# SensorsINI/v2e

Hardware: NVIDIA H100
Metric: Mevents/s (higher is better)
Workload: dtype fp16 tensor-core convs (fp32 accumulate) + f64 pixel state

## Files before the change

include/v2e_b200.h:

```cpp
#ifndef V2E_B200_H
#define V2E_B200_H

#include <stdint.h>

#ifdef __cplusplus
extern "C" {
#endif

typedef enum V2eStatus {
    V2E_OK = 0,
    V2E_E_INVALID = -1,
    V2E_E_CUDA = -2,
    V2E_E_CAPACITY = -3,
    V2E_E_ITER_CAP = -4,
    V2E_E_STATE = -5,
    V2E_E_UNSUPPORTED = -6,
    V2E_E_FALLBACK = -7
} V2eStatus;

typedef enum V2eFrameDtype { V2E_U8 = 0, V2E_F32 = 1, V2E_F64 = 2 } V2eFrameDtype;

const char *v2e_last_error(void);
int v2e_version(void);
int v2e_abi_info(int *version, int *emu_cfg_size, int *frame_info_size, int *unet_weights_size);
// ... 149 lines not shown
};
int v2e_conv2d_lrelu_sm100_tile(const void *x1_dev, int C1, const void *x2_dev, int C2,
                                const void *wgt_dev, const float *bias_dev, int Cout_pad, int KH, int KW,
                                int N, int H, int W, void *out_dev, int out_cstride, int out_mode,
                                int co_real, float slope, int tile, void *stream);
int v2e_conv_pick_tile(int C1, int C2, int Cout_pad, int KH, int KW, int N, int H, int W, int n_sms);

int v2e_conv2d_lrelu_sm100_strip(const void *x1_dev, int C1, const void *x2_dev, int C2,
                                 const void *wgt_row_dev, const float *bias_dev, int Cout_pad, int KH,
                                 int KW, int N, int H, int W, void *out_dev, int out_cstride,
                                 int out_mode, int co_real, float slope, void *stream);
int v2e_conv_strip_pick_kc(int C1, int C2, int Cout_pad, int KH, int KW, int W);

enum {
    V2E_STRIP_CHAIN_AUTO = -1,
    V2E_STRIP_CHAIN_PAIRED = 0,
    V2E_STRIP_CHAIN_STACKED = 1
};
int v2e_conv2d_lrelu_sm100_strip_chain(const void *x1_dev, int C1, const void *x2_dev, int C2,
                                       const void *wgt_row_dev, const float *bias_dev, int Cout_pad, int KH,
                                       int KW, int N, int H, int W, void *out_dev, int out_cstride,
                                       int out_mode, int co_real, float slope, int chain, void *stream);
int v2e_conv_strip_pick_chain(int C1, int C2, int Cout_pad, int KH, int KW, int W);

int v2e_conv2d_up2_lrelu_sm100(const void *x_low_dev, int C, const void *wgt_fold_dev, const void *wgt_plain_dev,
                               const float *bias_dev, int Cout_pad, int N, int H_out, int W_out, void *out_dev,
                               int out_cstride, float slope, void *stream);
int v2e_conv_up2_fold_weights(const float *w_host, int cout, int cin, int Cout_pad, int C_pad, void *out_host);
int v2e_conv_up2_supported_c(int C, int Cout_pad, int W_out);

typedef struct V2eUNetWeights {
    const float *w[23];
    const float *b[23];
} V2eUNetWeights;

typedef struct V2eSlomo V2eSlomo;

int v2e_slomo_create(int H, int W, int max_batch, const V2eUNetWeights *flow,
                     const V2eUNetWeights *interp, V2eSlomo **out);
int v2e_slomo_destroy(V2eSlomo *h);
int v2e_slomo_set_pairs(V2eSlomo *h, const uint8_t *frames_u8_dev, int B, void *stream);
int v2e_slomo_max_flow(V2eSlomo *h, float *max_speed_host, void *stream);
int v2e_slomo_interp(V2eSlomo *h, double t, uint8_t *out_u8_dev, float *out_f32_dev, void *stream);
int v2e_slomo_check_finite(V2eSlomo *h, int *nonfinite_host, void *stream);
int v2e_slomo_set_option(V2eSlomo *h, int option, int value);
int v2e_slomo_profile(V2eSlomo *h, int enable);
// ... 71 lines not shown
```

v2e_b200/_lib.py:

```python
import ctypes
import os

from . import build as _build

_LIB = None


class V2eEmuCfg(ctypes.Structure):
    _fields_ = [
        ("width", ctypes.c_int32), ("height", ctypes.c_int32),
        ("per_pixel_thres", ctypes.c_int32), ("hdr", ctypes.c_int32),
        ("pos_thres_nominal", ctypes.c_double), ("neg_thres_nominal", ctypes.c_double),
        ("cutoff_hz", ctypes.c_double), ("leak_rate_hz", ctypes.c_double),
        ("leak_jitter_fraction", ctypes.c_double), ("refractory_period_s", ctypes.c_double),
        ("shot_noise_rate_hz", ctypes.c_double), ("shot_inten_factor", ctypes.c_double),
        ("rng_mode", ctypes.c_int32), ("iter_cap", ctypes.c_int32),
        ("seed", ctypes.c_uint64),
        ("csdvs", ctypes.c_int32), ("max_frames_per_step", ctypes.c_int32),
        ("cs_tau_p_s", ctypes.c_double), ("cs_tau_h_s", ctypes.c_double),
        ("scidvs", ctypes.c_int32), ("photoreceptor_noise", ctypes.c_int32),
        ("rng_pixel_offset", ctypes.c_uint32), ("full_frame_px", ctypes.c_uint32),
        ("own_row0", ctypes.c_int32), ("own_rows", ctypes.c_int32),
        ("cs_halo_rows", ctypes.c_int32), ("reserved1", ctypes.c_int32),
    ]
# ... 60 lines not shown
    "v2e_emu_cs_begin": (_i, [_vp, _vp, _i, _d, _d, _u64, _u64, ctypes.POINTER(_i), _vp]),
    "v2e_emu_cs_pack": (_i, [_vp, _vp]),
    "v2e_emu_cs_unpack_from": (_i, [_vp, _vp, _vp, _vp]),
    "v2e_emu_cs_send_dev": (_vp, [_vp]),
    "v2e_emu_cs_chunk": (_i, [_vp, _i, _i, _vp]),
    "v2e_emu_cs_max_dev": (_vp, [_vp]),
    "v2e_emu_cs_advance": (_i, [_vp, _i, _i, _vp]),
    "v2e_emu_cs_update": (_i, [_vp, _vp, _i, _vp, _vp, _vp]),
    "v2e_emu_phase_filter": (_i, [_vp, _d, _d, _u64, _i, _vp]),
    "v2e_emu_read_counts": (_i, [_vp, ctypes.POINTER(ctypes.c_int32), _vp, _i, _vp]),
    "v2e_emu_phase_shot": (_i, [_vp, _vp, _i, _d, _d, _vp, _u64, _vp]),
    "v2e_emu_phase_emit": (_i, [_vp, _d, _d, _vp, _u64, _vp]),
    "v2e_conv2d_lrelu_sm100": (_i, [_vp, _i, _vp, _i, _vp, _vp, _i, _i, _i, _i, _i, _i, _vp, _i, _i, _i,
                                    ctypes.c_float, _vp]),
    "v2e_conv2d_lrelu_sm100_tile": (_i, [_vp, _i, _vp, _i, _vp, _vp, _i, _i, _i, _i, _i, _i, _vp, _i, _i, _i,
                                         ctypes.c_float, _i, _vp]),
    "v2e_conv_pick_tile": (_i, [_i, _i, _i, _i, _i, _i, _i, _i, _i]),
    "v2e_conv2d_lrelu_sm100_strip": (_i, [_vp, _i, _vp, _i, _vp, _vp, _i, _i, _i, _i, _i, _i, _vp, _i, _i, _i,
                                          ctypes.c_float, _vp]),
    "v2e_conv_strip_pick_kc": (_i, [_i, _i, _i, _i, _i, _i]),
    "v2e_conv2d_lrelu_sm100_strip_chain": (_i, [_vp, _i, _vp, _i, _vp, _vp, _i, _i, _i, _i, _i, _i, _vp, _i, _i, _i,
                                                ctypes.c_float, _i, _vp]),
    "v2e_conv_strip_pick_chain": (_i, [_i, _i, _i, _i, _i, _i]),
    "v2e_conv2d_up2_lrelu_sm100": (_i, [_vp, _i, _vp, _vp, _vp, _i, _i, _i, _i, _vp, _i, ctypes.c_float, _vp]),
    "v2e_conv_up2_fold_weights": (_i, [_vp, _i, _i, _i, _i, _vp]),
    "v2e_conv_up2_supported_c": (_i, [_i, _i, _i]),
    "v2e_slomo_create": (_i, [_i, _i, _i, _vp, _vp, ctypes.POINTER(_vp)]),
    "v2e_slomo_destroy": (_i, [_vp]),
    "v2e_slomo_set_pairs": (_i, [_vp, _vp, _i, _vp]),
    "v2e_slomo_max_flow": (_i, [_vp, ctypes.POINTER(ctypes.c_float), _vp]),
    "v2e_slomo_interp": (_i, [_vp, _d, _vp, _vp, _vp]),
    "v2e_slomo_set_option": (_i, [_vp, _i, _i]),
    "v2e_slomo_check_finite": (_i, [_vp, ctypes.POINTER(_i), _vp]),
    "v2e_slomo_profile": (_i, [_vp, _i]),
    "v2e_slomo_profile_read": (_i, [_vp, ctypes.POINTER(ctypes.c_float), ctypes.POINTER(_i),
                                    ctypes.POINTER(ctypes.c_double), _vp]),
    "v2e_slomo_profile_read_layers": (_i, [_vp, ctypes.POINTER(ctypes.c_float), ctypes.POINTER(_i),
                                           ctypes.POINTER(ctypes.c_double), ctypes.POINTER(ctypes.c_float),
                                           ctypes.POINTER(_i), ctypes.POINTER(ctypes.c_double), _vp]),
    "v2e_slomo_flow_ptr": (_vp, [_vp]),
    "v2e_slomo_intrp_ptr": (_vp, [_vp]),
    "v2e_slomo_buffer_ptr": (_vp, [_vp, _i, _i]),
    "v2e_slomo_layer_kernel": (_i, [_vp, _i, _i]),
    "v2e_resize_create": (_i, [_i, _i, _i, _i, _i, _i, ctypes.POINTER(_vp)]),
    "v2e_resize_destroy": (_i, [_vp]),
    "v2e_resize_run": (_i, [_vp, _vp, _vp, _i, _vp]),
# ... 91 lines not shown
```

v2e_b200/csrc/conv_tc.cu:

```cuda
#include <cuda.h>
#include <cuda_fp16.h>
#include <cuda_runtime.h>
#include <math.h>
#include <stdint.h>
#include <stdio.h>
#include <string.h>
#include <vector>

#include "../../include/v2e_b200.h"
#include "common.cuh"
#include "tc_common.cuh"

namespace {

constexpr int kTileH = 8, kTileW = 16, kBM = kTileH * kTileW;
constexpr int kStages = 4;
constexpr int kConvThreads = 288;
constexpr int kProducerWarp = 8;
constexpr int kConsumerWarps = 8;

struct ConvParams {
    int N, H, W;
    int C1, C2;
    int KH, KW;
// ... 213 lines not shown
#pragma unroll
            for (int i = 0; i < 2; i++) {
                const int m = 64 * (g * MH + h) + 16 * (warp & 3) + (lane >> 2) + 8 * i;
                const int py = y0 + m / kTileW, px = x0 + m % kTileW;
                inb[i] = py < p.H && px < p.W;
                pix[i] = (((size_t)n * p.H + py) * p.W + px) * p.out_cstride;
            }
#pragma unroll
            for (int j = 0; j < BN / 8; j++) {
                const int c = 8 * j + 2 * (lane & 3);
                const float2 b = __ldg((const float2 *)(bias + c));
#pragma unroll
                for (int i = 0; i < 2; i++)
                    if (inb[i])
                        *(__half2 *)(out + pix[i] + c) = __floats2half2_rn(lrelu(acc[h][4 * j + 2 * i] + b.x, p.slope),
                                                                           lrelu(acc[h][4 * j + 2 * i + 1] + b.y, p.slope));
            }
        }
    }
}


constexpr int kRowTile = 128;

struct StripParams {
    int N, H, W;
    int C1, C2;
    int KH, KW;
    int KC, BN;
    int tiles_x, seg_h, n_seg, n_items;
    int nslot;
    void *pool_out;
    int pool_cstride;
    int n_split, cout_pad;
    int slab_bytes;
    int w_bytes;
    int out_cstride, out_mode, co_real;
    float slope;
    const float *bias;
    void *out;
};
constexpr int kMaxSlot = 12;
constexpr int kStripThreads = 288;

struct RowRing {
    uint64_t *full, *empty;
    uint32_t nslot, cnt;
    int waited, released;
    __device__ __forceinline__ uint32_t slot(int i) const { return (cnt + (uint32_t)i) % nslot; }
    __device__ __forceinline__ void wait_upto(int n) {
        for (; waited < n; waited++) {
            const uint32_t g = cnt + (uint32_t)waited;
            mbar_wait(&full[g % nslot], (g / nslot) & 1u);
        }
    }
    __device__ __forceinline__ void release_upto(int n, int lane) {
        wait_upto(n);
        __syncwarp();
        for (; released < n; released++)
            if (lane == 0) mbar_arrive(&empty[slot(released)]);
    }
};

template <int KW, int KC, int BN>
__device__ __forceinline__ void strip_pair_mma(float (&acc)[2][BN / 2], const RowRing &rr, int row0, int last, int slabs,
                                                uint64_t dr, uint64_t dw, uint32_t a_off, uint32_t row16, uint32_t slab16,
// ... 30 lines not shown
                                                 uint64_t dr, uint64_t dw, uint32_t a_off, uint32_t row16, uint32_t slab16,
                                                 int rp0, int rp1) {
    constexpr int KH = KW;
    constexpr uint32_t rowb16 = (KC * 2u) >> 4, tile16 = (BN * KC * 2u) >> 4, wslab16 = stack_tiles<KW>() * tile16;
#pragma unroll
    for (int rp = rp0; rp < rp1; rp++) {
        const uint32_t a_row = rr.slot(row0 + (rp < KH ? rp : last)) * row16 + a_off;
        int sl = 0;
#pragma unroll 1
        do {
            const uint32_t a_lo = a_row + (uint32_t)sl * slab16;
            const uint32_t w_lo = (uint32_t)sl * wslab16 + (uint32_t)stack_index<KW>(rp, 0) * tile16;
#pragma unroll
            for (int s = 0; s < KW; s++) {
#pragma unroll
                for (int j = 0; j < KC / 16; j++)
                    wgmma_f16<2 * BN>(acc, desc_add(dr, a_lo + (uint32_t)s * rowb16 + 2u * j),
                                      desc_add(dw, w_lo + (uint32_t)(s * (KH + 1)) * tile16 + 2u * j), 1u);
            }
        } while (++sl < slabs);
    }
}

template <int KW, int KC, int BN, bool POOL, bool STACK>
__global__ void __launch_bounds__(kStripThreads, 1)
conv_strip_kernel(const __grid_constant__ CUtensorMap tmA, const __grid_constant__ CUtensorMap tmA2,
                  const __grid_constant__ CUtensorMap tmB, const StripParams p) {
    extern __shared__ __align__(1024) uint8_t smem_raw[];
    uint8_t *smem = align1024(smem_raw);
    __shared__ __align__(8) uint64_t full_bar[kMaxSlot], empty_bar[kMaxSlot], w_bar;

    constexpr int KH = KW, ph = KH / 2, pw = KW / 2, taps = KH * KW;
    constexpr int PW = kRowTile + KW - 1;
    constexpr uint32_t tile_bytes = BN * KC * 2;
    const int warp = threadIdx.x >> 5, lane = threadIdx.x & 31;
    const int slabs = (p.C1 + p.C2) / KC;
    const uint32_t row_bytes = (uint32_t)p.slab_bytes * slabs;
    uint8_t *ring = smem + ((p.w_bytes + 1023) & ~1023);
    const int split = (int)blockIdx.x % p.n_split, co_off = split * BN;
    const int item0 = (int)blockIdx.x / p.n_split, item_step = (int)gridDim.x / p.n_split;

    if constexpr (STACK) {
        constexpr int z_vec = (int)tile_bytes / 16, z_per_slab = KW + 1;
        for (int i = threadIdx.x; i < slabs * z_per_slab * z_vec; i += blockDim.x) {
            const int z = i / z_vec, sl = z / z_per_slab, s = z % z_per_slab;
            ((uint4 *)(smem + ((size_t)sl * stack_tiles<KW>() + (size_t)s * (KH + 1)) * tile_bytes))[i % z_vec] =
                make_uint4(0u, 0u, 0u, 0u);
        }
        fence_proxy_async();
    }
    if (threadIdx.x == 0) {
        for (int s = 0; s < p.nslot; s++) { mbar_init(&full_bar[s], 1); mbar_init(&empty_bar[s], kConsumerWarps); }
        mbar_init(&w_bar, 1);
        fence_barrier_init();
    }
    if (warp == kProducerWarp && lane == 0) {
        prefetch_tmap(&tmA);
        if (p.C2) prefetch_tmap(&tmA2);
        prefetch_tmap(&tmB);
    }
    __syncthreads();

    if (warp == kProducerWarp) {
        if (lane == 0) {
            mbar_expect_tx(&w_bar, (uint32_t)(slabs * taps) * tile_bytes);
            for (int t = 0; t < slabs * taps; t++) {
                const int sl = t / taps, tap = t % taps;
                const int dst = STACK ? sl * stack_tiles<KW>() + stack_index<KW>(tap / KW, tap % KW) : t;
                tma_load_2d(smem + (size_t)dst * tile_bytes, &tmB, &w_bar, 0, t * p.cout_pad + co_off);
            }
            uint32_t cnt = 0;
            for (int item = item0; item < p.n_items; item += item_step) {
                const int tx = item % p.tiles_x, rest = item / p.tiles_x;
                const int seg = rest % p.n_seg, n = rest / p.n_seg;
                const int ya = seg * p.seg_h, yb = min(p.H, ya + p.seg_h);
                const int x0 = tx * kRowTile;
                for (int i = ya - ph; i < yb + ph; i++, cnt++) {
                    const int slot = (int)(cnt % (uint32_t)p.nslot);
                    mbar_wait(&empty_bar[slot], ((cnt / (uint32_t)p.nslot) & 1u) ^ 1u);
                    mbar_expect_tx(&full_bar[slot], (uint32_t)(PW * KC * 2 * slabs));
                    uint8_t *dst = ring + (size_t)slot * row_bytes;
                    for (int sl = 0; sl < slabs; sl++) {
                        const int c = sl * KC;
                        if (c < p.C1) tma_load_4d(dst + (size_t)sl * p.slab_bytes, &tmA, &full_bar[slot], c, x0 - pw, i, n);
                        else tma_load_4d(dst + (size_t)sl * p.slab_bytes, &tmA2, &full_bar[slot], c - p.C1, x0 - pw, i, n);
                    }
                }
            }
        }
    } else {
        const int g = __shfl_sync(0xffffffffu, warp >> 2, 0);
        constexpr uint32_t sbo = 8u * KC * 2u, half16 = (64u * KC * 2u) >> 4;
        constexpr bool kOverlap = BN <= 32;
        const uint64_t dw = make_smem_desc(smem_u32(smem), swizzle_layout(KC), sbo);
        const uint64_t dr = make_smem_desc(smem_u32(ring), swizzle_layout(KC), sbo);
        const uint32_t row16 = row_bytes >> 4, slab16 = (uint32_t)p.slab_bytes >> 4;
        mbar_wait(&w_bar, 0);
        RowRing rr{full_bar, empty_bar, (uint32_t)p.nslot, 0u, 0, 0};
        for (int item = item0; item < p.n_items; item += item_step) {
            const int tx = item % p.tiles_x, rest = item / p.tiles_x;
            const int seg = rest % p.n_seg, n = rest / p.n_seg;
            const int ya = seg * p.seg_h, yb = min(p.H, ya + p.seg_h);
            const int rows_out = yb - ya, rows_in = rows_out + 2 * ph;
            rr.waited = 0; rr.released = 0;
            for (int q = g; 2 * q < rows_out; q += 2) {
                rr.release_upto(2 * q, lane);
                const bool two = 2 * q + 1 < rows_out;
                rr.wait_upto(2 * q + KH + (two ? 1 : 0));
                float acc[2][BN];
                auto rows = [&](int hf) -> float (&)[2][BN / 2] { return *reinterpret_cast<float (*)[2][BN / 2]>(acc[hf]); };
                auto zero = [&](int hf) {
#pragma unroll
                    for (int i = 0; i < BN; i++) acc[hf][i] = 0.f;
                    wgmma_fence_regs(acc[hf]);
                };
                auto issue = [&](int hf, int rp0, int rp1) {
                    if constexpr (STACK)
                        strip_stack_mma<KW, KC, BN>(acc[hf], rr, 2 * q, two ? KH : KH - 1, slabs, dr, dw, hf * half16,
                                                     row16, slab16, rp0, rp1);
                    else
                        strip_pair_mma<KW, KC, BN>(rows(hf), rr, 2 * q, two ? KH : KH - 1, slabs, dr, dw, hf * half16,
                                                    row16, slab16, rp0, rp1);
                };
                const int y = ya + 2 * q;
                auto epilogue = [&](int hf) {
#pragma unroll
                    for (int i = 0; i < 2; i++) {
                        const int m = 64 * hf + 16 * (warp & 3) + (lane >> 2) + 8 * i;
                        const int px = tx * kRowTile + m;
                        const bool inb = px < p.W;
                        const size_t pix = ((size_t)n * p.H + y) * p.W + px;
                        __half2 h0[BN / 8], h1[BN / 8];
                        epilogue_row<BN>(rows(hf)[0], i, inb, pix, lane, p.bias + co_off, p.slope, p.out_mode, p.out,
                                         p.out_cstride, co_off, h0);
                        if (two) {
                            epilogue_row<BN>(rows(hf)[1], i, inb, pix + p.W, lane, p.bias + co_off, p.slope, p.out_mode, p.out,
                                             p.out_cstride, co_off, h1);
                            if (POOL) {
                                __half2 *pl = (__half2 *)((__half *)p.pool_out +
                                    (((size_t)n * (p.H / 2) + y / 2) * (p.W / 2) + px / 2) * p.pool_cstride + co_off);
#pragma unroll
                                for (int j = 0; j < BN / 8; j++) {
                                    const float2 a = __half22float2(h1[j]), b = __half22float2(h0[j]);
                                    float s0 = a.x + b.x, s1 = a.y + b.y;
                                    s0 += __shfl_xor_sync(0xffffffffu, s0, 4);
                                    s1 += __shfl_xor_sync(0xffffffffu, s1, 4);
                                    if (inb && (lane & 4) == 0)
                                        pl[(8 * j + 2 * (lane & 3)) / 2] = __floats2half2_rn(s0 * 0.25f, s1 * 0.25f);
                                }
                            }
                        }
                    }
                };
                if constexpr (kOverlap) {
                    zero(0);
                    zero(1);
                    wgmma_fence();
                    issue(0, 0, 2);
                    issue(1, 0, 2);
                    wgmma_commit();
                    issue(0, 2, KH + 1);
                    wgmma_commit();
                    issue(1, 2, KH + 1);
                    wgmma_commit();
                    wgmma_wait<2>();
                    rr.release_upto(2 * q + 2, lane);
                    wgmma_wait<1>();
                    wgmma_fence_regs(acc[0]);
                    epilogue(0);
                    wgmma_wait<0>();
                    wgmma_fence_regs(acc[1]);
                    rr.release_upto(min(rows_in, 2 * q + 4), lane);
                    epilogue(1);
                } else {
#pragma unroll
                    for (int hf = 0; hf < 2; hf++) {
                        zero(hf);
                        wgmma_fence();
                        issue(hf, 0, KH + 1);
                        wgmma_commit();
                        wgmma_wait<0>();
                        wgmma_fence_regs(acc[hf]);
                        if (hf == 1) rr.release_upto(min(rows_in, 2 * q + 4), lane);
                        epilogue(hf);
                    }
                }
            }
            rr.release_upto(rows_in, lane);
            rr.cnt += (uint32_t)rows_in;
        }
    }
}

constexpr int kUpBlocks = 6;

__global__ void __launch_bounds__(kStripThreads, 1)
// ... 371 lines not shown
    V2eConvLaunch L;
    int rc = v2e_conv_prepare(&L, x1_dev, C1, x2_dev, C2, wgt_dev, bias_dev, Cout_pad, KH, KW, N, H, W, out_dev,
                              out_cstride, out_mode, co_real, slope, tile, device_sms());
    if (rc) return rc;
    return v2e_conv_launch(&L, (cudaStream_t)stream);
}

extern "C" int v2e_conv2d_lrelu_sm100(const void *x1_dev, int C1, const void *x2_dev, int C2,
                                      const void *wgt_dev, const float *bias_dev, int Cout_pad, int KH, int KW,
                                      int N, int H, int W, void *out_dev, int out_cstride, int out_mode,
                                      int co_real, float slope, void *stream) {
    return v2e_conv2d_lrelu_sm100_tile(x1_dev, C1, x2_dev, C2, wgt_dev, bias_dev, Cout_pad, KH, KW, N, H, W, out_dev,
                                       out_cstride, out_mode, co_real, slope, V2E_CONV_TILE_AUTO, stream);
}

struct V2eStripLaunch {
    CUtensorMap tmA, tmA2, tmB;
    StripParams p;
    int stacked;
    int grid;
    size_t smem;
};

static int make_rowseg_tmap(CUtensorMap *tm, const void *ptr, int N, int H, int W, int C, int KC, int KW) {
    EncodeTiledFn fn = encode_fn();
    if (!fn) return v2e_set_error(V2E_E_CUDA, "cuTensorMapEncodeTiled unavailable%s", "");
    cuuint64_t dims[4] = {(cuuint64_t)C, (cuuint64_t)W, (cuuint64_t)H, (cuuint64_t)N};
    cuuint64_t strides[3] = {(cuuint64_t)C * 2, (cuuint64_t)W * C * 2, (cuuint64_t)H * W * C * 2};
    cuuint32_t box[4] = {(cuuint32_t)KC, (cuuint32_t)(kRowTile + KW - 1), 1, 1};
    cuuint32_t es[4] = {1, 1, 1, 1};
    CUresult r = fn(tm, CU_TENSOR_MAP_DATA_TYPE_FLOAT16, 4, (void *)ptr, dims, strides, box, es,
                    CU_TENSOR_MAP_INTERLEAVE_NONE, swizzle_for(KC), CU_TENSOR_MAP_L2_PROMOTION_L2_256B,
                    CU_TENSOR_MAP_FLOAT_OOB_FILL_NONE);
    if (r != CUDA_SUCCESS) return v2e_set_error(V2E_E_CUDA, "cuTensorMapEncodeTiled failed for a strip row map%s", "");
    return V2E_OK;
}

constexpr size_t kSmemFull = 222 * 1024, kSmemHalf = 110 * 1024;

static size_t strip_w_bytes(int slabs, int KH, int KW, int bn, int kc, int stacked) {
    return (size_t)slabs * (stacked ? KW * (KH + 1) + 1 : KH * KW) * bn * kc * 2;
}

static int strip_config(int C1, int C2, int Cout_pad, int KH, int KW, int kc, int stacked, int *nslot, int *ctas_per_sm,
                        int *n_split) {
    if (Cout_pad > 64) return 0;
    const int slabs = (C1 + C2) / kc;
    const size_t row = (((size_t)(kRowTile + KW - 1) * kc * 2 + 1023) & ~(size_t)1023) * slabs;
    for (int split = 1; split <= 2; split++) {
        const int bn = Cout_pad / split;
        if (bn < 16 || bn % 16) break;
        const size_t wb = (strip_w_bytes(slabs, KH, KW, bn, kc, stacked) + 1023) & ~(size_t)1023;
        const int two = wb + 2048 + (size_t)(KH + 3) * row <= kSmemHalf;
        const size_t budget = two ? kSmemHalf : kSmemFull;
        if (wb + 2048 + (size_t)(KH + 1) * row > budget) continue;
        int ns = (int)((budget - wb - 2048) / row);
        if (ns > kMaxSlot) ns = kMaxSlot;
        *nslot = ns; *ctas_per_sm = two ? 2 : 1; *n_split = split;
        return 1;
    }
    return 0;
}

constexpr int kStripMinW = 2 * kRowTile;

int v2e_strip_pick(int C1, int C2, int Cout_pad, int KH, int KW, int W, int *nslot_out) {
    if (Cout_pad > 64 || KH != KW || W < kStripMinW || (KW != 3 && KW != 5 && KW != 7)) return 0;
    const int g = C2 ? (C1 < C2 ? C1 : C2) : C1;
    const int kc = g % 64 == 0 ? 64 : (g % 32 == 0 ? 32 : 16);
    int ns, cps, nsp;
    if (!strip_config(C1, C2, Cout_pad, KH, KW, kc, 0, &ns, &cps, &nsp)) return 0;
    if (nslot_out) *nslot_out = ns;
    return kc;
}

static int strip_auto_stacked(int C1, int C2, int Cout_pad, int KH, int KW, int kc) {
    int ns0, cps0, nsp0, ns1, cps1, nsp1;
    if (!strip_config(C1, C2, Cout_pad, KH, KW, kc, 0, &ns0, &cps0, &nsp0) || Cout_pad / nsp0 > 32 ||
        !strip_config(C1, C2, Cout_pad, KH, KW, kc, 1, &ns1, &cps1, &nsp1))
        return 0;
    return cps1 == cps0 && nsp1 == nsp0;
}

static int strip_plan(int C1, int C2, int Cout_pad, int KH, int KW, int kc, int chain, int *nslot, int *ctas_per_sm,
                      int *n_split, int *stacked) {
    *stacked = chain == V2E_STRIP_CHAIN_AUTO ? strip_auto_stacked(C1, C2, Cout_pad, KH, KW, kc)
                                             : chain == V2E_STRIP_CHAIN_STACKED;
    return strip_config(C1, C2, Cout_pad, KH, KW, kc, *stacked, nslot, ctas_per_sm, n_split);
}

extern "C" int v2e_conv_strip_pick_chain(int C1, int C2, int Cout_pad, int KH, int KW, int W) {
    const int kc = v2e_strip_pick(C1, C2, Cout_pad, KH, KW, W, nullptr);
    return kc ? strip_auto_stacked(C1, C2, Cout_pad, KH, KW, kc) : -1;
}

size_t v2e_strip_launch_size(void) { return sizeof(V2eStripLaunch); }

static bool strip_pool_ok(int KW, int KC, int H, int W, int ctas_per_sm, int bn) {
    return !(H & 1) && !(W & 1) && ((KW == 7 && KC == 32) || (KW == 5 && KC == 64)) && ctas_per_sm == 1 && bn >= 32;
}

int v2e_strip_pool_supported(int C1, int C2, int Cout_pad, int KH, int KW, int H, int W) {
    const int KC = v2e_strip_pick(C1, C2, Cout_pad, KH, KW, W, nullptr);
    int ns, cps, nsp, st;
    if (!KC || !strip_plan(C1, C2, Cout_pad, KH, KW, KC, V2E_STRIP_CHAIN_AUTO, &ns, &cps, &nsp, &st)) return 0;
    return strip_pool_ok(KW, KC, H, W, cps, Cout_pad / nsp);
}

int v2e_strip_prepare(V2eStripLaunch *L, const void *x1, int C1, const void *x2, int C2, const void *wgt_row,
                      const float *bias, int Cout_pad, int KH, int KW, int N, int H, int W, void *out,
                      int out_cstride, int out_mode, int co_real, float slope, int n_sms, void *pool_out,
                      int pool_cstride, int chain) {
    memset(L, 0, sizeof(*L));
    StripParams &p = L->p;
    if (chain < V2E_STRIP_CHAIN_AUTO || chain > V2E_STRIP_CHAIN_STACKED)
        return v2e_set_error(V2E_E_INVALID, "strip: unknown chain%s", "");
    const int KC = v2e_strip_pick(C1, C2, Cout_pad, KH, KW, W, nullptr);
    int nslot = 0, ctas_per_sm = 0, n_split = 0, stacked = 0;
    if (!KC || !strip_plan(C1, C2, Cout_pad, KH, KW, KC, chain, &nslot, &ctas_per_sm, &n_split, &stacked))
        return v2e_set_error(V2E_E_INVALID, "layer does not qualify for the strip kernel (with this chain)%s", "");
    L->stacked = stacked;
    p.N = N; p.H = H; p.W = W; p.C1 = C1; p.C2 = C2; p.KH = KH; p.KW = KW; p.KC = KC;
    p.n_split = n_split; p.cout_pad = Cout_pad; p.BN = Cout_pad / n_split;
    p.tiles_x = (W + kRowTile - 1) / kRowTile;
    int seg_h = H;
    const int strips = p.tiles_x * N;
    while (seg_h > 4 * KH && (long)strips * ((H + seg_h - 1) / seg_h) < 6L * n_sms) seg_h = (seg_h + 1) / 2;
    if (pool_out) {
        if (out_mode != 0 || !strip_pool_ok(KW, KC, H, W, ctas_per_sm, p.BN))
            return v2e_set_error(V2E_E_UNSUPPORTED, "strip: this layer has no pooled epilogue%s", "");
        seg_h = (seg_h + 1) & ~1;
    }
    p.pool_out = pool_out;
    p.pool_cstride = pool_cstride;
    p.seg_h = seg_h;
    p.n_seg = (H + seg_h - 1) / seg_h;
    p.n_items = strips * p.n_seg;
    p.nslot = nslot;
    const int slabs = (C1 + C2) / KC, taps = KH * KW;
    p.slab_bytes = (int)(((size_t)(kRowTile + KW - 1) * KC * 2 + 1023) & ~(size_t)1023);
    p.w_bytes = (int)strip_w_bytes(slabs, KH, KW, p.BN, KC, stacked);
    p.out_cstride = out_cstride; p.out_mode = out_mode; p.co_real = co_real; p.slope = slope;
    p.bias = bias; p.out = out;
    int rc;
    if ((rc = make_rowseg_tmap(&L->tmA, x1, N, H, W, C1, KC, KW))) return rc;
    if (C2) { if ((rc = make_rowseg_tmap(&L->tmA2, x2, N, H, W, C2, KC, KW))) return rc; }
    else L->tmA2 = L->tmA;
    {
        EncodeTiledFn fn = encode_fn();
        const int rows_total = slabs * taps * Cout_pad;
        cuuint64_t dims[2] = {(cuuint64_t)KC, (cuuint64_t)rows_total};
        cuuint64_t strides[1] = {(cuuint64_t)KC * 2};
        cuuint32_t box[2] = {(cuuint32_t)KC, (cuuint32_t)p.BN};
        cuuint32_t es[2] = {1, 1};
        CUresult r = fn(&L->tmB, CU_TENSOR_MAP_DATA_TYPE_FLOAT16, 2, (void *)wgt_row, dims, strides, box, es,
                        CU_TENSOR_MAP_INTERLEAVE_NONE, swizzle_for(KC), CU_TENSOR_MAP_L2_PROMOTION_L2_256B,
                        CU_TENSOR_MAP_FLOAT_OOB_FILL_NONE);
        if (r != CUDA_SUCCESS) return v2e_set_error(V2E_E_CUDA, "cuTensorMapEncodeTiled failed for strip weights%s", "");
    }
    L->smem = (size_t)((p.w_bytes + 1023) & ~1023) + (size_t)p.nslot * p.slab_bytes * slabs + 1024;
    int per = ctas_per_sm * n_sms / p.n_split;
    if (per > p.n_items) per = p.n_items;
    if (per < 1) per = 1;
    L->grid = per * p.n_split;
    return V2E_OK;
}

template <int KW, int KC, int BN, bool POOL, bool STACK>
static cudaError_t strip_launch_s(const V2eStripLaunch *L, cudaStream_t st) {
    static PerDeviceOnce attr_once;
    if (attr_once.first())
        cudaFuncSetAttribute(conv_strip_kernel<KW, KC, BN, POOL, STACK>, cudaFuncAttributeMaxDynamicSharedMemorySize, 226 * 1024);
    conv_strip_kernel<KW, KC, BN, POOL, STACK><<<L->grid, kStripThreads, L->smem, st>>>(L->tmA, L->tmA2, L->tmB, L->p);
    return cudaGetLastError();
}

template <int KW, int KC, int BN, bool POOL>
static cudaError_t strip_launch_t(const V2eStripLaunch *L, cudaStream_t st) {
    return L->stacked ? strip_launch_s<KW, KC, BN, POOL, true>(L, st) : strip_launch_s<KW, KC, BN, POOL, false>(L, st);
}

template <int KW, int KC>
static int strip_launch_kc(const V2eStripLaunch *L, cudaStream_t st, cudaError_t *e) {
    const StripParams &p = L->p;
    if (p.KW != KW || p.KC != KC) return 0;
    if (p.pool_out) {
        if constexpr ((KW == 7 && KC == 32) || (KW == 5 && KC == 64)) {
            if (p.BN == 32) { *e = strip_launch_t<KW, KC, 32, true>(L, st); return 1; }
            if (p.BN == 64) { *e = strip_launch_t<KW, KC, 64, true>(L, st); return 1; }
        }
        return 0;
    }
    if (p.BN == 16) { *e = strip_launch_t<KW, KC, 16, false>(L, st); return 1; }
    if (p.BN == 32) { *e = strip_launch_t<KW, KC, 32, false>(L, st); return 1; }
    if (p.BN == 64) { *e = strip_launch_t<KW, KC, 64, false>(L, st); return 1; }
    return 0;
}

int v2e_strip_launch(const V2eStripLaunch *L, cudaStream_t st) {
    cudaError_t e = cudaSuccess;
    const int launched = strip_launch_kc<3, 16>(L, st, &e) || strip_launch_kc<3, 32>(L, st, &e) ||
                         strip_launch_kc<3, 64>(L, st, &e) || strip_launch_kc<5, 16>(L, st, &e) ||
// ... 21 lines not shown

extern "C" int v2e_conv2d_lrelu_sm100_strip(const void *x1_dev, int C1, const void *x2_dev, int C2,
                                            const void *wgt_row_dev, const float *bias_dev, int Cout_pad, int KH,
                                            int KW, int N, int H, int W, void *out_dev, int out_cstride,
                                            int out_mode, int co_real, float slope, void *stream) {
    return v2e_conv2d_lrelu_sm100_strip_chain(x1_dev, C1, x2_dev, C2, wgt_row_dev, bias_dev, Cout_pad, KH, KW, N, H, W,
                                              out_dev, out_cstride, out_mode, co_real, slope, V2E_STRIP_CHAIN_AUTO, stream);
}


struct V2eUpLaunch {
    CUtensorMap tmA, tmB;
    StripParams p;
    int grid;
    size_t smem;
    const __half *low;
    const __half *w_plain;
    int C;
};

int v2e_conv_up2_supported(int C, int Cout_pad, int W_out) {
    if (C != 64 || Cout_pad != 32 || W_out % 2 || W_out < 2 * kStripMinW) return 0;
    const size_t wb = (size_t)(C / 64) * 2 * 3 * kUpBlocks * Cout_pad * 64 * 2;
    const size_t slab = ((size_t)(kRowTile + 2) * 64 * 2 + 1023) & ~(size_t)1023;
    return wb + 2048 + 3 * slab * (C / 64) <= kSmemFull;
}

extern "C" int v2e_conv_up2_fold_weights(const float *w, int cout, int cin, int Cout_pad, int C_pad, void *out_host) {
    if (!w || !out_host || C_pad % 64 || cin > C_pad || cout > Cout_pad) return v2e_set_error(V2E_E_INVALID, "bad argument%s", "");
    __half *o = (__half *)out_host;
    auto coef = [](int i, int a) -> float {
        const int t = i >= 0 ? i / 2 : -((1 - i) / 2), odd = i - 2 * t;
        if (!odd) return a == t - 1 ? 0.25f : (a == t ? 0.75f : 0.f);
        return a == t ? 0.75f : (a == t + 1 ? 0.25f : 0.f);
    };
    const int slabs = C_pad / 64;
    for (int sl = 0; sl < slabs; sl++)
        for (int px = 0; px < 2; px++)
            for (int b = 0; b < 3; b++)
                for (int q = 0; q < kUpBlocks; q++) {
                    const int py = q & 1, a = 1 - (q >> 1);
                    for (int co = 0; co < Cout_pad; co++)
                        for (int c = 0; c < 64; c++) {
                            const int ci = sl * 64 + c;
                            float v = 0.f;
                            if (co < cout && ci < cin)
                                for (int r = 0; r < 3; r++)
// ... 7 lines not shown

size_t v2e_conv_up2_launch_size(void) { return sizeof(V2eUpLaunch); }

int v2e_conv_up2_prepare(V2eUpLaunch *L, const void *x_low, int C, const void *wgt_fold, const void *wgt_plain,
                         const float *bias, int Cout_pad, int N, int H, int W, void *out, int out_cstride, float slope,
                         int n_sms) {
    memset(L, 0, sizeof(*L));
    if (!v2e_conv_up2_supported(C, Cout_pad, W) || H % 2) return v2e_set_error(V2E_E_INVALID, "layer does not qualify for the fused up-sampling convolution%s", "");
    if (!(slope >= 0.f && slope <= 1.f)) return v2e_set_error(V2E_E_INVALID, "slope must be in [0, 1]%s", "");
    StripParams &p = L->p;
    const int hl = H / 2, wl = W / 2, KC = 64;
    p.N = N; p.H = H; p.W = W; p.C1 = C; p.C2 = 0; p.KH = 3; p.KW = 3; p.KC = KC; p.BN = Cout_pad;
    p.tiles_x = (wl + kRowTile - 1) / kRowTile;
    const int strips = p.tiles_x * N;
    int n_seg = (6 * n_sms + strips - 1) / strips;
    if (n_seg < 1) n_seg = 1;
    int seg_h = (hl + n_seg - 1) / n_seg;
    if (seg_h < 8) seg_h = hl < 8 ? hl : 8;
    p.seg_h = seg_h;
    p.n_seg = (hl + seg_h - 1) / seg_h;
    p.n_items = strips * p.n_seg;
    p.n_split = 1; p.cout_pad = Cout_pad;
    const int slabs = C / KC;
    p.slab_bytes = (int)(((size_t)(kRowTile + 2) * KC * 2 + 1023) & ~(size_t)1023);
    p.w_bytes = slabs * 2 * 3 * kUpBlocks * Cout_pad * KC * 2;
    const int rows_total = slabs * 2 * 3 * kUpBlocks * Cout_pad;
    int ns = (int)((kSmemFull - (size_t)p.w_bytes - 2048) / ((size_t)p.slab_bytes * slabs));
    if (ns > kMaxSlot) ns = kMaxSlot;
    if (ns < 3) return v2e_set_error(V2E_E_INVALID, "fused up-sampling convolution: weights leave no room for the input ring%s", "");
    p.nslot = ns;
    p.out_cstride = out_cstride; p.out_mode = 0; p.co_real = Cout_pad; p.slope = slope;
    p.bias = bias; p.out = out;
    int rc;
    if ((rc = make_rowseg_tmap(&L->tmA, x_low, N, hl, wl, C, KC, 3))) return rc;
    {
        EncodeTiledFn fn = encode_fn();
        cuuint64_t dims[2] = {(cuuint64_t)KC, (cuuint64_t)rows_total};
        cuuint64_t strides[1] = {(cuuint64_t)KC * 2};
        cuuint32_t box[2] = {(cuuint32_t)KC, (cuuint32_t)(2 * Cout_pad)};
        cuuint32_t es[2] = {1, 1};
        CUresult r = fn(&L->tmB, CU_TENSOR_MAP_DATA_TYPE_FLOAT16, 2, (void *)wgt_fold, dims, strides, box, es,
                        CU_TENSOR_MAP_INTERLEAVE_NONE, swizzle_for(KC), CU_TENSOR_MAP_L2_PROMOTION_L2_256B,
                        CU_TENSOR_MAP_FLOAT_OOB_FILL_NONE);
        if (r != CUDA_SUCCESS) return v2e_set_error(V2E_E_CUDA, "cuTensorMapEncodeTiled failed for folded weights%s", "");
    }
    L->smem = (size_t)((p.w_bytes + 1023) & ~1023) + (size_t)p.nslot * p.slab_bytes * slabs + 1024;
    L->grid = p.n_items < n_sms ? p.n_items : n_sms;
    L->low = (const __half *)x_low;
    L->w_plain = (const __half *)wgt_plain;
    L->C = C;
    return V2E_OK;
}

int v2e_conv_up2_launch(const V2eUpLaunch *L, cudaStream_t st) {
    static PerDeviceOnce attr_once;
    if (attr_once.first()) cudaFuncSetAttribute(conv_up2_kernel, cudaFuncAttributeMaxDynamicSharedMemorySize, 226 * 1024);
    conv_up2_kernel<<<L->grid, kStripThreads, L->smem, st>>>(L->tmA, L->tmB, L->p);
// ... 30 lines not shown
```

Before: 57.39.

## Add 64-pixel row-tile strip variant with three consumer warpgroups for split layers

For strip convolutions whose output channels are split (BN <= 32), the planner may now pick a 64-pixel row tile instead of 128 when shared memory still fits enough ring slots. The kernel is templated on the row tile: with 64-pixel strips it runs three consumer warpgroups, each handling one half-tile per row pair, and the TMA box, slab size and ring release schedule are adjusted to match. The aim is more parallel work items and deeper row pipelining for narrow layers. In exchange, each item reuses weights over a narrower strip, the halo overhead per pixel is larger, and another template instantiation is compiled. A plan query entry point is also exposed.

```diff
diff --git a/include/v2e_b200.h b/include/v2e_b200.h
--- a/include/v2e_b200.h
+++ b/include/v2e_b200.h
@@ -195,6 +195,7 @@
                                        int KW, int N, int H, int W, void *out_dev, int out_cstride,
                                        int out_mode, int co_real, float slope, int chain, void *stream);
 int v2e_conv_strip_pick_chain(int C1, int C2, int Cout_pad, int KH, int KW, int W);
+int v2e_conv_strip_plan(int C1, int C2, int Cout_pad, int KH, int KW, int W, int chain, int *plan);
 
 int v2e_conv2d_up2_lrelu_sm100(const void *x_low_dev, int C, const void *wgt_fold_dev, const void *wgt_plain_dev,
                                const float *bias_dev, int Cout_pad, int N, int H_out, int W_out, void *out_dev,
diff --git a/v2e_b200/_lib.py b/v2e_b200/_lib.py
--- a/v2e_b200/_lib.py
+++ b/v2e_b200/_lib.py
@@ -106,6 +106,7 @@
     "v2e_conv2d_lrelu_sm100_strip_chain": (_i, [_vp, _i, _vp, _i, _vp, _vp, _i, _i, _i, _i, _i, _i, _vp, _i, _i, _i,
                                                 ctypes.c_float, _i, _vp]),
     "v2e_conv_strip_pick_chain": (_i, [_i, _i, _i, _i, _i, _i]),
+    "v2e_conv_strip_plan": (_i, [_i, _i, _i, _i, _i, _i, _i, ctypes.POINTER(ctypes.c_int)]),
     "v2e_conv2d_up2_lrelu_sm100": (_i, [_vp, _i, _vp, _vp, _vp, _i, _i, _i, _i, _vp, _i, ctypes.c_float, _vp]),
     "v2e_conv_up2_fold_weights": (_i, [_vp, _i, _i, _i, _i, _vp]),
     "v2e_conv_up2_supported_c": (_i, [_i, _i, _i]),
diff --git a/v2e_b200/csrc/conv_tc.cu b/v2e_b200/csrc/conv_tc.cu
--- a/v2e_b200/csrc/conv_tc.cu
+++ b/v2e_b200/csrc/conv_tc.cu
@@ -259,6 +259,7 @@
 
 
 constexpr int kRowTile = 128;
+constexpr int kRowTileSplit = 64;
 
 struct StripParams {
     int N, H, W;
@@ -266,6 +267,7 @@
     int KH, KW;
     int KC, BN;
     int tiles_x, seg_h, n_seg, n_items;
+    int row_tile;
     int nslot;
     void *pool_out;
     int pool_cstride;
@@ -279,6 +281,10 @@
 };
 constexpr int kMaxSlot = 12;
 constexpr int kStripThreads = 288;
+template <int RT>
+__host__ __device__ constexpr int strip_warpgroups() { return RT == 64 ? 3 : 2; }
+template <int RT>
+__host__ __device__ constexpr int strip_threads() { return 32 * (4 * strip_warpgroups<RT>() + 1); }
 
 struct RowRing {
     uint64_t *full, *empty;
@@ -355,8 +361,8 @@
     }
 }
 
-template <int KW, int KC, int BN, bool POOL, bool STACK>
-__global__ void __launch_bounds__(kStripThreads, 1)
+template <int KW, int KC, int BN, bool POOL, bool STACK, int RT>
+__global__ void __launch_bounds__(strip_threads<RT>(), 1)
 conv_strip_kernel(const __grid_constant__ CUtensorMap tmA, const __grid_constant__ CUtensorMap tmA2,
                   const __grid_constant__ CUtensorMap tmB, const StripParams p) {
     extern __shared__ __align__(1024) uint8_t smem_raw[];
@@ -364,7 +370,7 @@
     __shared__ __align__(8) uint64_t full_bar[kMaxSlot], empty_bar[kMaxSlot], w_bar;
 
     constexpr int KH = KW, ph = KH / 2, pw = KW / 2, taps = KH * KW;
-    constexpr int PW = kRowTile + KW - 1;
+    constexpr int PW = RT + KW - 1, HALVES = RT / 64, NWG = strip_warpgroups<RT>(), producer = 4 * NWG;
     constexpr uint32_t tile_bytes = BN * KC * 2;
     const int warp = threadIdx.x >> 5, lane = threadIdx.x & 31;
     const int slabs = (p.C1 + p.C2) / KC;
@@ -383,18 +389,18 @@
         fence_proxy_async();
     }
     if (threadIdx.x == 0) {
-        for (int s = 0; s < p.nslot; s++) { mbar_init(&full_bar[s], 1); mbar_init(&empty_bar[s], kConsumerWarps); }
+        for (int s = 0; s < p.nslot; s++) { mbar_init(&full_bar[s], 1); mbar_init(&empty_bar[s], 4 * NWG); }
         mbar_init(&w_bar, 1);
         fence_barrier_init();
     }
-    if (warp == kProducerWarp && lane == 0) {
+    if (warp == producer && lane == 0) {
         prefetch_tmap(&tmA);
         if (p.C2) prefetch_tmap(&tmA2);
         prefetch_tmap(&tmB);
     }
     __syncthreads();
 
-    if (warp == kProducerWarp) {
+    if (warp == producer) {
         if (lane == 0) {
             mbar_expect_tx(&w_bar, (uint32_t)(slabs * taps) * tile_bytes);
             for (int t = 0; t < slabs * taps; t++) {
@@ -407,7 +413,7 @@
                 const int tx = item % p.tiles_x, rest = item / p.tiles_x;
                 const int seg = rest % p.n_seg, n = rest / p.n_seg;
                 const int ya = seg * p.seg_h, yb = min(p.H, ya + p.seg_h);
-                const int x0 = tx * kRowTile;
+                const int x0 = tx * RT;
                 for (int i = ya - ph; i < yb + ph; i++, cnt++) {
                     const int slot = (int)(cnt % (uint32_t)p.nslot);
                     mbar_wait(&empty_bar[slot], ((cnt / (uint32_t)p.nslot) & 1u) ^ 1u);
@@ -425,6 +431,7 @@
         const int g = __shfl_sync(0xffffffffu, warp >> 2, 0);
         constexpr uint32_t sbo = 8u * KC * 2u, half16 = (64u * KC * 2u) >> 4;
         constexpr bool kOverlap = BN <= 32;
+        static_assert(HALVES == 2 || (HALVES == 1 && kOverlap), "64-pixel strips: split layers (BN <= 32) only");
         const uint64_t dw = make_smem_desc(smem_u32(smem), swizzle_layout(KC), sbo);
         const uint64_t dr = make_smem_desc(smem_u32(ring), swizzle_layout(KC), sbo);
         const uint32_t row16 = row_bytes >> 4, slab16 = (uint32_t)p.slab_bytes >> 4;
@@ -436,11 +443,11 @@
             const int ya = seg * p.seg_h, yb = min(p.H, ya + p.seg_h);
             const int rows_out = yb - ya, rows_in = rows_out + 2 * ph;
             rr.waited = 0; rr.released = 0;
-            for (int q = g; 2 * q < rows_out; q += 2) {
+            for (int q = g; 2 * q < rows_out; q += NWG) {
                 rr.release_upto(2 * q, lane);
                 const bool two = 2 * q + 1 < rows_out;
                 rr.wait_upto(2 * q + KH + (two ? 1 : 0));
-                float acc[2][BN];
+                float acc[HALVES][BN];
                 auto rows = [&](int hf) -> float (&)[2][BN / 2] { return *reinterpret_cast<float (*)[2][BN / 2]>(acc[hf]); };
                 auto zero = [&](int hf) {
 #pragma unroll
@@ -460,7 +467,7 @@
 #pragma unroll
                     for (int i = 0; i < 2; i++) {
                         const int m = 64 * hf + 16 * (warp & 3) + (lane >> 2) + 8 * i;
-                        const int px = tx * kRowTile + m;
+                        const int px = tx * RT + m;
                         const bool inb = px < p.W;
                         const size_t pix = ((size_t)n * p.H + y) * p.W + px;
                         __half2 h0[BN / 8], h1[BN / 8];
@@ -486,25 +493,28 @@
                     }
                 };
                 if constexpr (kOverlap) {
-                    zero(0);
-                    zero(1);
+#pragma unroll
+                    for (int hf = 0; hf < HALVES; hf++) zero(hf);
                     wgmma_fence();
-                    issue(0, 0, 2);
-                    issue(1, 0, 2);
+#pragma unroll
+                    for (int hf = 0; hf < HALVES; hf++) issue(hf, 0, 2);
                     wgmma_commit();
-                    issue(0, 2, KH + 1);
-                    wgmma_commit();
-                    issue(1, 2, KH + 1);
-                    wgmma_commit();
-                    wgmma_wait<2>();
+#pragma unroll
+                    for (int hf = 0; hf < HALVES; hf++) {
+                        issue(hf, 2, KH + 1);
+                        wgmma_commit();
+                    }
+                    wgmma_wait<HALVES>();
                     rr.release_upto(2 * q + 2, lane);
-                    wgmma_wait<1>();
-                    wgmma_fence_regs(acc[0]);
-                    epilogue(0);
+                    if constexpr (HALVES == 2) {
+                        wgmma_wait<1>();
+                        wgmma_fence_regs(acc[0]);
+                        epilogue(0);
+                    }
                     wgmma_wait<0>();
-                    wgmma_fence_regs(acc[1]);
-                    rr.release_upto(min(rows_in, 2 * q + 4), lane);
-                    epilogue(1);
+                    wgmma_fence_regs(acc[HALVES - 1]);
+                    rr.release_upto(min(rows_in, 2 * (q + NWG)), lane);
+                    epilogue(HALVES - 1);
                 } else {
 #pragma unroll
                     for (int hf = 0; hf < 2; hf++) {
@@ -922,12 +932,12 @@
     size_t smem;
 };
 
-static int make_rowseg_tmap(CUtensorMap *tm, const void *ptr, int N, int H, int W, int C, int KC, int KW) {
+static int make_rowseg_tmap(CUtensorMap *tm, const void *ptr, int N, int H, int W, int C, int KC, int KW, int row_tile) {
     EncodeTiledFn fn = encode_fn();
     if (!fn) return v2e_set_error(V2E_E_CUDA, "cuTensorMapEncodeTiled unavailable%s", "");
     cuuint64_t dims[4] = {(cuuint64_t)C, (cuuint64_t)W, (cuuint64_t)H, (cuuint64_t)N};
     cuuint64_t strides[3] = {(cuuint64_t)C * 2, (cuuint64_t)W * C * 2, (cuuint64_t)H * W * C * 2};
-    cuuint32_t box[4] = {(cuuint32_t)KC, (cuuint32_t)(kRowTile + KW - 1), 1, 1};
+    cuuint32_t box[4] = {(cuuint32_t)KC, (cuuint32_t)(row_tile + KW - 1), 1, 1};
     cuuint32_t es[4] = {1, 1, 1, 1};
     CUresult r = fn(tm, CU_TENSOR_MAP_DATA_TYPE_FLOAT16, 4, (void *)ptr, dims, strides, box, es,
                     CU_TENSOR_MAP_INTERLEAVE_NONE, swizzle_for(KC), CU_TENSOR_MAP_L2_PROMOTION_L2_256B,
@@ -942,21 +952,37 @@
     return (size_t)slabs * (stacked ? KW * (KH + 1) + 1 : KH * KW) * bn * kc * 2;
 }
 
+static size_t strip_slab_bytes(int row_tile, int KW, int kc) {
+    return ((size_t)(row_tile + KW - 1) * kc * 2 + 1023) & ~(size_t)1023;
+}
+
+static int strip_ring(size_t wb, size_t row_bytes, int KH, int *nslot, int *ctas_per_sm) {
+    const int two = wb + 2048 + (size_t)(KH + 3) * row_bytes <= kSmemHalf;
+    const size_t budget = two ? kSmemHalf : kSmemFull;
+    if (wb + 2048 + (size_t)(KH + 1) * row_bytes > budget) return 0;
+    const int ns = (int)((budget - wb - 2048) / row_bytes);
+    *nslot = ns < kMaxSlot ? ns : kMaxSlot;
+    *ctas_per_sm = two ? 2 : 1;
+    return 1;
+}
+
 static int strip_config(int C1, int C2, int Cout_pad, int KH, int KW, int kc, int stacked, int *nslot, int *ctas_per_sm,
-                        int *n_split) {
+                        int *n_split, int *row_tile) {
     if (Cout_pad > 64) return 0;
     const int slabs = (C1 + C2) / kc;
-    const size_t row = (((size_t)(kRowTile + KW - 1) * kc * 2 + 1023) & ~(size_t)1023) * slabs;
     for (int split = 1; split <= 2; split++) {
         const int bn = Cout_pad / split;
         if (bn < 16 || bn % 16) break;
         const size_t wb = (strip_w_bytes(slabs, KH, KW, bn, kc, stacked) + 1023) & ~(size_t)1023;
-        const int two = wb + 2048 + (size_t)(KH + 3) * row <= kSmemHalf;
-        const size_t budget = two ? kSmemHalf : kSmemFull;
-        if (wb + 2048 + (size_t)(KH + 1) * row > budget) continue;
-        int ns = (int)((budget - wb - 2048) / row);
-        if (ns > kMaxSlot) ns = kMaxSlot;
-        *nslot = ns; *ctas_per_sm = two ? 2 : 1; *n_split = split;
+        if (!strip_ring(wb, strip_slab_bytes(kRowTile, KW, kc) * slabs, KH, nslot, ctas_per_sm)) continue;
+        *n_split = split;
+        *row_tile = kRowTile;
+        if (split > 1) {
+            const size_t budget = *ctas_per_sm == 2 ? kSmemHalf : kSmemFull;
+            int ns = (int)((budget - wb - 2048) / (strip_slab_bytes(kRowTileSplit, KW, kc) * slabs));
+            if (ns > kMaxSlot) ns = kMaxSlot;
+            if (ns >= KH + 3) { *nslot = ns; *row_tile = kRowTileSplit; }
+        }
         return 1;
     }
     return 0;
@@ -968,25 +994,25 @@
     if (Cout_pad > 64 || KH != KW || W < kStripMinW || (KW != 3 && KW != 5 && KW != 7)) return 0;
     const int g = C2 ? (C1 < C2 ? C1 : C2) : C1;
     const int kc = g % 64 == 0 ? 64 : (g % 32 == 0 ? 32 : 16);
-    int ns, cps, nsp;
-    if (!strip_config(C1, C2, Cout_pad, KH, KW, kc, 0, &ns, &cps, &nsp)) return 0;
+    int ns, cps, nsp, rt;
+    if (!strip_config(C1, C2, Cout_pad, KH, KW, kc, 0, &ns, &cps, &nsp, &rt)) return 0;
     if (nslot_out) *nslot_out = ns;
     return kc;
 }
 
 static int strip_auto_stacked(int C1, int C2, int Cout_pad, int KH, int KW, int kc) {
-    int ns0, cps0, nsp0, ns1, cps1, nsp1;
-    if (!strip_config(C1, C2, Cout_pad, KH, KW, kc, 0, &ns0, &cps0, &nsp0) || Cout_pad / nsp0 > 32 ||
-        !strip_config(C1, C2, Cout_pad, KH, KW, kc, 1, &ns1, &cps1, &nsp1))
+    int ns0, cps0, nsp0, rt0, ns1, cps1, nsp1, rt1;
+    if (!strip_config(C1, C2, Cout_pad, KH, KW, kc, 0, &ns0, &cps0, &nsp0, &rt0) || Cout_pad / nsp0 > 32 ||
+        !strip_config(C1, C2, Cout_pad, KH, KW, kc, 1, &ns1, &cps1, &nsp1, &rt1))
         return 0;
     return cps1 == cps0 && nsp1 == nsp0;
 }
 
 static int strip_plan(int C1, int C2, int Cout_pad, int KH, int KW, int kc, int chain, int *nslot, int *ctas_per_sm,
-                      int *n_split, int *stacked) {
+                      int *n_split, int *stacked, int *row_tile) {
     *stacked = chain == V2E_STRIP_CHAIN_AUTO ? strip_auto_stacked(C1, C2, Cout_pad, KH, KW, kc)
                                              : chain == V2E_STRIP_CHAIN_STACKED;
-    return strip_config(C1, C2, Cout_pad, KH, KW, kc, *stacked, nslot, ctas_per_sm, n_split);
+    return strip_config(C1, C2, Cout_pad, KH, KW, kc, *stacked, nslot, ctas_per_sm, n_split, row_tile);
 }
 
 extern "C" int v2e_conv_strip_pick_chain(int C1, int C2, int Cout_pad, int KH, int KW, int W) {
@@ -994,6 +1020,16 @@
     return kc ? strip_auto_stacked(C1, C2, Cout_pad, KH, KW, kc) : -1;
 }
 
+extern "C" int v2e_conv_strip_plan(int C1, int C2, int Cout_pad, int KH, int KW, int W, int chain, int *plan) {
+    const int kc = v2e_strip_pick(C1, C2, Cout_pad, KH, KW, W, nullptr);
+    int ns, cps, nsp, st, rt;
+    if (!kc || chain < V2E_STRIP_CHAIN_AUTO || chain > V2E_STRIP_CHAIN_STACKED ||
+        !strip_plan(C1, C2, Cout_pad, KH, KW, kc, chain, &ns, &cps, &nsp, &st, &rt))
+        return 0;
+    plan[0] = rt; plan[1] = ns; plan[2] = cps; plan[3] = nsp; plan[4] = st;
+    return 1;
+}
+
 size_t v2e_strip_launch_size(void) { return sizeof(V2eStripLaunch); }
 
 static bool strip_pool_ok(int KW, int KC, int H, int W, int ctas_per_sm, int bn) {
@@ -1002,8 +1038,8 @@
 
 int v2e_strip_pool_supported(int C1, int C2, int Cout_pad, int KH, int KW, int H, int W) {
     const int KC = v2e_strip_pick(C1, C2, Cout_pad, KH, KW, W, nullptr);
-    int ns, cps, nsp, st;
-    if (!KC || !strip_plan(C1, C2, Cout_pad, KH, KW, KC, V2E_STRIP_CHAIN_AUTO, &ns, &cps, &nsp, &st)) return 0;
+    int ns, cps, nsp, st, rt;
+    if (!KC || !strip_plan(C1, C2, Cout_pad, KH, KW, KC, V2E_STRIP_CHAIN_AUTO, &ns, &cps, &nsp, &st, &rt)) return 0;
     return strip_pool_ok(KW, KC, H, W, cps, Cout_pad / nsp);
 }
 
@@ -1016,13 +1052,14 @@
     if (chain < V2E_STRIP_CHAIN_AUTO || chain > V2E_STRIP_CHAIN_STACKED)
         return v2e_set_error(V2E_E_INVALID, "strip: unknown chain%s", "");
     const int KC = v2e_strip_pick(C1, C2, Cout_pad, KH, KW, W, nullptr);
-    int nslot = 0, ctas_per_sm = 0, n_split = 0, stacked = 0;
-    if (!KC || !strip_plan(C1, C2, Cout_pad, KH, KW, KC, chain, &nslot, &ctas_per_sm, &n_split, &stacked))
+    int nslot = 0, ctas_per_sm = 0, n_split = 0, stacked = 0, row_tile = 0;
+    if (!KC || !strip_plan(C1, C2, Cout_pad, KH, KW, KC, chain, &nslot, &ctas_per_sm, &n_split, &stacked, &row_tile))
         return v2e_set_error(V2E_E_INVALID, "layer does not qualify for the strip kernel (with this chain)%s", "");
     L->stacked = stacked;
     p.N = N; p.H = H; p.W = W; p.C1 = C1; p.C2 = C2; p.KH = KH; p.KW = KW; p.KC = KC;
     p.n_split = n_split; p.cout_pad = Cout_pad; p.BN = Cout_pad / n_split;
-    p.tiles_x = (W + kRowTile - 1) / kRowTile;
+    p.row_tile = row_tile;
+    p.tiles_x = (W + row_tile - 1) / row_tile;
     int seg_h = H;
     const int strips = p.tiles_x * N;
     while (seg_h > 4 * KH && (long)strips * ((H + seg_h - 1) / seg_h) < 6L * n_sms) seg_h = (seg_h + 1) / 2;
@@ -1038,13 +1075,13 @@
     p.n_items = strips * p.n_seg;
     p.nslot = nslot;
     const int slabs = (C1 + C2) / KC, taps = KH * KW;
-    p.slab_bytes = (int)(((size_t)(kRowTile + KW - 1) * KC * 2 + 1023) & ~(size_t)1023);
+    p.slab_bytes = (int)strip_slab_bytes(row_tile, KW, KC);
     p.w_bytes = (int)strip_w_bytes(slabs, KH, KW, p.BN, KC, stacked);
     p.out_cstride = out_cstride; p.out_mode = out_mode; p.co_real = co_real; p.slope = slope;
     p.bias = bias; p.out = out;
     int rc;
-    if ((rc = make_rowseg_tmap(&L->tmA, x1, N, H, W, C1, KC, KW))) return rc;
-    if (C2) { if ((rc = make_rowseg_tmap(&L->tmA2, x2, N, H, W, C2, KC, KW))) return rc; }
+    if ((rc = make_rowseg_tmap(&L->tmA, x1, N, H, W, C1, KC, KW, row_tile))) return rc;
+    if (C2) { if ((rc = make_rowseg_tmap(&L->tmA2, x2, N, H, W, C2, KC, KW, row_tile))) return rc; }
     else L->tmA2 = L->tmA;
     {
         EncodeTiledFn fn = encode_fn();
@@ -1066,18 +1103,27 @@
     return V2E_OK;
 }
 
-template <int KW, int KC, int BN, bool POOL, bool STACK>
+template <int KW, int KC, int BN, bool POOL, bool STACK, int RT>
 static cudaError_t strip_launch_s(const V2eStripLaunch *L, cudaStream_t st) {
     static PerDeviceOnce attr_once;
     if (attr_once.first())
-        cudaFuncSetAttribute(conv_strip_kernel<KW, KC, BN, POOL, STACK>, cudaFuncAttributeMaxDynamicSharedMemorySize, 226 * 1024);
-    conv_strip_kernel<KW, KC, BN, POOL, STACK><<<L->grid, kStripThreads, L->smem, st>>>(L->tmA, L->tmA2, L->tmB, L->p);
+        cudaFuncSetAttribute(conv_strip_kernel<KW, KC, BN, POOL, STACK, RT>, cudaFuncAttributeMaxDynamicSharedMemorySize,
+                             226 * 1024);
+    conv_strip_kernel<KW, KC, BN, POOL, STACK, RT><<<L->grid, strip_threads<RT>(), L->smem, st>>>(L->tmA, L->tmA2, L->tmB,
+                                                                                              L->p);
     return cudaGetLastError();
+}
+
+template <int KW, int KC, int BN, bool POOL, bool STACK>
+static cudaError_t strip_launch_w(const V2eStripLaunch *L, cudaStream_t st) {
+    if constexpr (BN <= 32)
+        if (L->p.row_tile == kRowTileSplit) return strip_launch_s<KW, KC, BN, POOL, STACK, kRowTileSplit>(L, st);
+    return strip_launch_s<KW, KC, BN, POOL, STACK, kRowTile>(L, st);
 }
 
 template <int KW, int KC, int BN, bool POOL>
 static cudaError_t strip_launch_t(const V2eStripLaunch *L, cudaStream_t st) {
-    return L->stacked ? strip_launch_s<KW, KC, BN, POOL, true>(L, st) : strip_launch_s<KW, KC, BN, POOL, false>(L, st);
+    return L->stacked ? strip_launch_w<KW, KC, BN, POOL, true>(L, st) : strip_launch_w<KW, KC, BN, POOL, false>(L, st);
 }
 
 template <int KW, int KC>
@@ -1145,7 +1191,7 @@
 int v2e_conv_up2_supported(int C, int Cout_pad, int W_out) {
     if (C != 64 || Cout_pad != 32 || W_out % 2 || W_out < 2 * kStripMinW) return 0;
     const size_t wb = (size_t)(C / 64) * 2 * 3 * kUpBlocks * Cout_pad * 64 * 2;
-    const size_t slab = ((size_t)(kRowTile + 2) * 64 * 2 + 1023) & ~(size_t)1023;
+    const size_t slab = strip_slab_bytes(kRowTile, 3, 64);
     return wb + 2048 + 3 * slab * (C / 64) <= kSmemFull;
 }
 
@@ -1199,7 +1245,7 @@
     p.n_items = strips * p.n_seg;
     p.n_split = 1; p.cout_pad = Cout_pad;
     const int slabs = C / KC;
-    p.slab_bytes = (int)(((size_t)(kRowTile + 2) * KC * 2 + 1023) & ~(size_t)1023);
+    p.slab_bytes = (int)strip_slab_bytes(kRowTile, 3, KC);
     p.w_bytes = slabs * 2 * 3 * kUpBlocks * Cout_pad * KC * 2;
     const int rows_total = slabs * 2 * 3 * kUpBlocks * Cout_pad;
     int ns = (int)((kSmemFull - (size_t)p.w_bytes - 2048) / ((size_t)p.slab_bytes * slabs));
@@ -1209,7 +1255,7 @@
     p.out_cstride = out_cstride; p.out_mode = 0; p.co_real = Cout_pad; p.slope = slope;
     p.bias = bias; p.out = out;
     int rc;
-    if ((rc = make_rowseg_tmap(&L->tmA, x_low, N, hl, wl, C, KC, 3))) return rc;
+    if ((rc = make_rowseg_tmap(&L->tmA, x_low, N, hl, wl, C, KC, 3, kRowTile))) return rc;
     {
         EncodeTiledFn fn = encode_fn();
         cuuint64_t dims[2] = {(cuuint64_t)KC, (cuuint64_t)rows_total};
```

Result: faster. 58.52 (median of 6 runs) (+2.0%).
